# CognitiveAISystems/pogema

Measured on AMD Instinct MI355X. Metric: agent-steps/sec (whole node), 64-agent 64x64 grid, batch=8192 envs, higher is better.
Workload: dtype u32

## Files before the change

### include/pogema_amd.h

```cpp
#ifndef POGEMA_AMD_H
#define POGEMA_AMD_H

#include <stddef.h>
#include <stdint.h>

#ifdef __cplusplus
extern "C" {
#endif

#define PGX_ABI_VERSION 6

#define PGX_OK 0
#define PGX_E_INVALID (-1)
#define PGX_E_HIP (-2)
#define PGX_E_NOMEM (-3)
#define PGX_E_STATE (-4)
#define PGX_E_PLACEMENT (-5)

#define PGX_COLLISION_PRIORITY 0
#define PGX_COLLISION_BLOCK_BOTH 1
#define PGX_COLLISION_SOFT 2

#define PGX_ON_TARGET_FINISH 0
#define PGX_ON_TARGET_RESTART 1
// ... 67 lines not shown
int pgx_regenerate(pgx_env* env, const uint8_t* env_mask, float density, uint64_t seed, const uint8_t* shared_map,
                   int32_t max_retries, void* obs, void* stream);
int64_t pgx_regenerate_failures(pgx_env* env, void* stream);

int pgx_set_map_pool(pgx_env* env, const uint8_t* maps, int32_t num_maps, int32_t* capacity_out, void* stream);
int pgx_reset_pool(pgx_env* env, uint64_t seed, const uint8_t* env_mask, int32_t max_retries, void* stream);
int pgx_regenerate_pool(pgx_env* env, const uint8_t* env_mask, uint64_t seed, int32_t max_retries, void* obs,
                        void* stream);
int pgx_get_map_index(pgx_env* env, int32_t* map_index, void* stream);

int pgx_get_map(pgx_env* env, uint8_t* obstacles, void* stream);

int pgx_step(pgx_env* env, const void* actions, int action_dtype, void* obs, float* rewards,
             uint8_t* terminated, uint8_t* truncated, uint8_t* is_active, void* stream);

int pgx_xcd_shares(pgx_env* env, int32_t* shares);
int pgx_xcd_tune(pgx_env* env, void* obs, void* obs_alt, int32_t rounds, float* us_equal, float* us_tuned, void* stream);

typedef struct pgx_geometry {
    int32_t lanes_per_env;
    int32_t waves;
    int32_t envs_per_wave;
    int32_t multi_wave;
    int32_t p16;
    int32_t stagger;
    int32_t store_policy;
    int32_t state_stores;
    int32_t grid;
    int32_t lds_bytes;
    int32_t for_rollout;
// ... 142 lines not shown
```

### pogema_amd/_lib.py

```python
from __future__ import annotations

import ctypes as C
import os

_HERE = os.path.dirname(os.path.abspath(__file__))
LIB_PATH = os.environ.get("PGX_LIB") or os.path.join(_HERE, "libpogema_amd.so")

PGX_ABI_VERSION = 6

COLLISION_SYSTEMS = {"priority": 0, "block_both": 1, "soft": 2}
ON_TARGET = {"finish": 0, "restart": 1, "nothing": 2}
ACTION_DTYPES = {"int8": 0, "int32": 1, "int64": 2}
SOFT_VERTEX_RULES = {"lowest_index": 0, "all_stay": 1}
SOFT_OCCUPANCY = {"index_order": 0, "exact": 1}
COOP_REWARDS = {"all_solved": 0, "per_agent": 1}
BAD_ACTIONS = {"noop": 0, "flag": 1}
LIFELONG_RNGS = {"build": 0, "numpy": 1}
def _obs_dtypes():
    import torch
    return {torch.float32: 0, torch.uint8: 1, torch.bfloat16: 2, torch.float16: 3}


def obs_elem_bytes(dtype) -> int:
    import torch
# ... 20 lines not shown
MAX_OBS_RADIUS, MAX_AGENTS, MAX_SIDE = 15, 1024, 1024
MAX_NEIGHBOURS = 32
DIRECTIONS_FORMATS = {"float32": 0, "uint8": 1, "bits": 2}
SHIELD_TIE_BREAKS = {None: 0, "distance": 1}
MAX_PLAN_HORIZON = 256
PLAN_FIXED_PRIORITY = 1
OUTCOMES = ("STAY", "MOVED", "OBSTACLE", "SWAP", "OCCUPIED", "FOLLOW", "CONTESTED")
NUM_OUTCOMES = len(OUTCOMES)
POLICY_CHANNELS = {"obstacles": 0, "agents": 1, "target": 2, "other_goals": 3, "up": 4, "down": 5, "left": 6, "right": 7}
NUM_CHANNELS = len(POLICY_CHANNELS)
DEFAULT_POLICY_CHANNELS = ("obstacles", "agents", "target", "up", "down", "left", "right")


EXPORTED_SYMBOLS = (
    "pgx_abi_version", "pgx_last_error", "pgx_create", "pgx_check_config", "pgx_destroy", "pgx_obs_elems", "pgx_agent_elems",
    "pgx_reset_from_state", "pgx_reset_random", "pgx_regenerate", "pgx_regenerate_failures", "pgx_get_map", "pgx_step", "pgx_observe", "pgx_set_metrics_buffers", "pgx_get_state", "pgx_generate", "pgx_place_agents",
    "pgx_snapshot_bytes", "pgx_save_snapshot", "pgx_load_snapshot", "pgx_time_observe", "pgx_bad_action_count",
    "pgx_buffers_create", "pgx_buffers_ptr", "pgx_buffers_get_info", "pgx_buffers_destroy", "pgx_set_targets",
    "pgx_np_streams", "pgx_np_streams_host", "pgx_np_generate", "pgx_np_generate_host", "pgx_rollout", "pgx_buffers_stride", "pgx_buffers_drop", "pgx_xcd_shares", "pgx_xcd_tune", "pgx_buffers_create_at", "pgx_time_observe_pair", "pgx_buffers_va_reserved", "pgx_get_geometry",
    "pgx_expert_actions", "pgx_set_map_pool", "pgx_reset_pool", "pgx_regenerate_pool", "pgx_get_map_index",
    "pgx_cost_to_go", "pgx_cost_to_go_bytes", "pgx_cost_to_go_builds", "pgx_visible_agents", "pgx_pibt_actions",
    "pgx_goal_directions", "pgx_shield_actions", "pgx_pibt_plan", "pgx_move_outcomes",
    "pgx_policy_input",
)


class PgxError(RuntimeError):
    def __init__(self, code: int, message: str):
        super().__init__(f"pogema_amd engine error {code}: {message}")
        self.code = code

# ... 124 lines not shown
    lib.pgx_get_map_index.restype = C.c_int
    lib.pgx_set_targets.argtypes = [vp, vp, vp, vp]
    lib.pgx_set_targets.restype = C.c_int
    lib.pgx_bad_action_count.argtypes = [vp, vp]
    lib.pgx_bad_action_count.restype = i64
    lib.pgx_time_observe.argtypes = [vp, vp, i32, C.POINTER(C.c_float), vp]
    lib.pgx_time_observe.restype = C.c_int
    lib.pgx_time_observe_pair.argtypes = [vp, vp, vp, i32, C.POINTER(C.c_float), vp]
    lib.pgx_time_observe_pair.restype = C.c_int
    lib.pgx_snapshot_bytes.argtypes = [vp]
    lib.pgx_snapshot_bytes.restype = i64
    lib.pgx_save_snapshot.argtypes = [vp, vp, vp]
    lib.pgx_load_snapshot.argtypes = [vp, vp, vp]
    lib.pgx_save_snapshot.restype = lib.pgx_load_snapshot.restype = C.c_int
    lib.pgx_step.argtypes = [vp, vp, C.c_int, vp, vp, vp, vp, vp, vp]
    lib.pgx_observe.argtypes = [vp, vp, vp]
    lib.pgx_set_metrics_buffers.argtypes = [vp, vp, vp]
    lib.pgx_get_state.argtypes = [vp, vp, vp, vp, vp, vp, vp]
    lib.pgx_generate.argtypes = [i32, i32, i32, i32, f32, u64, i64, i32, i32, vp, vp, vp]
    lib.pgx_place_agents.argtypes = [i32, i32, i32, i32, u64, i64, i32, i32, vp, i32, vp, vp]
    for name in ("pgx_create", "pgx_destroy", "pgx_reset_from_state", "pgx_reset_random", "pgx_regenerate", "pgx_get_map",
                 "pgx_step", "pgx_observe", "pgx_set_metrics_buffers", "pgx_set_metrics_buffers",
                 "pgx_get_state", "pgx_generate", "pgx_place_agents"):
        getattr(lib, name).restype = C.c_int
    if lib.pgx_abi_version() != PGX_ABI_VERSION:
        raise ImportError(f"{LIB_PATH}: ABI version {lib.pgx_abi_version()} != expected {PGX_ABI_VERSION}; rebuild")
    _lib = lib
    return lib


# ... 5 lines not shown
```

### pogema_amd/buffers.py

```python
from __future__ import annotations

import atexit
import collections
import contextlib
import ctypes as C
import os
import threading

import numpy as np
import torch

from . import _lib

_TYPESTR = {torch.float32: "<f4", torch.uint8: "|u1", torch.float16: "<f2", torch.bfloat16: "<f2"}


class _Owner:

    def __init__(self, lib, handle):
        self._lib, self._handle = lib, handle

    def __del__(self):
        try:
            if self._handle is not None and self._handle.value:
# ... 320 lines not shown
        self._count = storage_count_hook()
        self._zone_ptrs = frozenset(int(p) for p in zone_ptrs)
        dev = obs_tensors[0].device
        n = batch * agents
        self._sets = []
        for obs in obs_tensors:
            block = torch.empty(n * 7 + 16, dtype=torch.uint8, device=dev)
            members = (obs, block[:4 * n].view(torch.float32).view(batch, agents),
                       block[4 * n:5 * n].view(torch.bool).view(batch, agents),
                       block[5 * n:6 * n].view(torch.bool).view(batch, agents),
                       block[6 * n:7 * n].view(torch.bool).view(batch, agents))
            storages = (obs.untyped_storage(), block.untyped_storage())
            self._sets.append((members, storages, tuple(st._cdata for st in storages)))
        del obs, block, members, storages
        self._idle = [tuple(self._count(c) for c in cdata) for _, _, cdata in self._sets]
        self._next = 0
        self.taken = 0
        self.misses = 0

    def __len__(self):
        return len(self._sets)

    def obs_pointers(self):
        return [members[0].data_ptr() for members, _, _ in self._sets]

    def _is_idle(self, i: int) -> bool:
        cdata, idle = self._sets[i][2], self._idle[i]
        return self._count(cdata[0]) == idle[0] and self._count(cdata[1]) == idle[1]

    def free_sets(self) -> int:
        return sum(self._is_idle(i) for i in range(len(self._sets)))

    def retire(self):
        idle = [i for i in range(len(self._sets)) if self._is_idle(i)]
        out = [self._sets[i][0][0] for i in idle if self._sets[i][0][0].data_ptr() in self._zone_ptrs]
        for i in reversed(idle):
            del self._sets[i]
            del self._idle[i]
        self._next = 0
        return out

    def take(self, with_obs: bool = True):
        n = len(self._sets)
        for k in range(n):
            i = (self._next + k) % n
            if self._is_idle(i):
                self._next = (i + 1) % n
                self.taken += 1
                m = self._sets[i][0]
                return (m[0].detach() if with_obs else None, m[1].detach(), m[2].detach(), m[3].detach(), m[4].detach())
        self.misses += 1
        return None
```

### pogema_amd/csrc/pgx_api.cpp

```cpp
#include "../../include/pogema_amd.h"

#include <hip/hip_runtime.h>

#include <algorithm>
#include <cstdarg>
#include <cstdio>
#include <cstdlib>
#include <cstring>
#include <new>
#include <string>
#include <vector>

#include "pgx_internal.h"

namespace {
thread_local std::string g_err;
}

namespace pgx {
int fail_msg(int code, const char* fmt, ...) {
    char buf[512];
    va_list ap;
    va_start(ap, fmt);
    vsnprintf(buf, sizeof buf, fmt, ap);
// ... 346 lines not shown
        alloc(e->comp_len, cells * sizeof(uint32_t));
        alloc(e->comp_cells, cells * sizeof(uint32_t));
        alloc(e->tcount, BA * sizeof(uint32_t));
        if (cfg->lifelong_rng == PGX_LIFELONG_RNG_NUMPY) {
            alloc(e->np_state, BA * sizeof(pgx::NpGen));
            alloc(e->np_state0, BA * sizeof(pgx::NpGen));
        }
    }
    if (err != hipSuccess) return fail_msg(alloc_code(err), "hipMalloc failed: %s", hipGetErrorString(err));
    err = hipMemset(e->regen_fail, 0, sizeof(uint32_t));
    if (err == hipSuccess) err = hipMemset(e->bad_count, 0, sizeof(uint32_t));
    if (err == hipSuccess && e->np_state0)
        err = pgx::launch_init_np_lifelong(e->np_state0, cfg->seed, cfg->env_index_base, cfg->batch, A, nullptr);
    if (err == hipSuccess && e->np_state0) err = hipStreamSynchronize(nullptr);
    if (err == hipSuccess) err = pgx::prepare_step(e->geo, e->geo_roll);
    if (err != hipSuccess)
        return fail_msg(PGX_E_HIP, "cannot configure the step kernel (%zu bytes of LDS): %s", e->geo.lds_bytes,
                        hipGetErrorString(err));
    if (const char* spec = getenv("PGX_XCD_WEIGHTS")) {
        float f[8], sum = 0.f;
        if (sscanf(spec, "%f,%f,%f,%f,%f,%f,%f,%f", &f[0], &f[1], &f[2], &f[3], &f[4], &f[5], &f[6], &f[7]) == 8) {
            for (float q : f) sum += q > 0.f ? q : 0.f;
            if (sum > 0.f)
                for (int x = 0; x < 8; ++x) e->xcd_w[x] = (f[x] > 0.f ? f[x] : 0.f) / sum;
        }
    }
    apply_xcd_shares(e);
    err = pgx::prepare_expert(cfg->height, cfg->width);
    if (err != hipSuccess) return fail_msg(PGX_E_HIP, "cannot configure the expert kernel: %s", hipGetErrorString(err));
    if (e->flags & 4u) {
// ... 458 lines not shown
             uint8_t* truncated, uint8_t* is_active, void* stream) {
    if (!e || !actions || !rewards || !terminated || !truncated) return fail_msg(PGX_E_INVALID, "pgx_step: null argument");
    if (const int rc = check_action_dtype("pgx_step", action_dtype)) return rc;
    DeviceGuard guard;
    if (const int rc = enter(guard, e, "pgx_step", true)) return rc;
    pgx::StepParams p = step_params(e, e->geo);
    p.mode = pgx::MODE_STEP;
    p.action_dtype = action_dtype;
    p.actions = actions;
    p.obs = static_cast<float*>(obs);
    p.rewards = rewards;
    p.terminated = terminated;
    p.truncated = truncated;
    p.act_out = is_active;
    PGX_HIP(pgx::launch_step(p, e->geo, (hipStream_t)stream));
    return PGX_OK;
}

int pgx_rollout(pgx_env* e, int32_t steps, const pgx_rollout_io* io, void* stream) {
    if (!e || !io || !io->rewards || !io->terminated || !io->truncated)
        return fail_msg(PGX_E_INVALID, "pgx_rollout: null argument");
    if (io->policy_step0 < 0 || io->policy_step0 > ((int64_t)1 << 40))
        return fail_msg(PGX_E_INVALID, "pgx_rollout: policy_step0 outside 0..2^40");
    if (steps < 1) return fail_msg(PGX_E_INVALID, "pgx_rollout: steps must be >= 1, got %d", steps);
    if (const int rc = check_action_dtype("pgx_rollout", io->action_dtype)) return rc;
    if (io->obs && io->obs_slots < 1) return fail_msg(PGX_E_INVALID, "pgx_rollout: obs given but obs_slots = %d", io->obs_slots);
    DeviceGuard guard;
    if (const int rc = enter(guard, e, "pgx_rollout", true)) return rc;
    pgx::StepParams p = step_params(e, e->geo_roll);
    p.mode = pgx::MODE_STEP;
// ... 514 lines not shown
```

### pogema_amd/csrc/pgx_internal.h

```cpp
#pragma once
#include <hip/hip_runtime.h>
#include <stddef.h>
#include <stdint.h>

namespace pgx {

int fail_msg(int code, const char* fmt, ...);

#define PGX_HIP(call)                                                                                                      \
    do {                                                                                                                   \
        const hipError_t e__ = (call);                                                                                     \
        if (e__ != hipSuccess)                                                                                             \
            return pgx::fail_msg(PGX_E_HIP, "%s failed: %s (%s:%d)", #call, hipGetErrorString(e__), __FILE__, __LINE__); \
    } while (0)

struct DeviceGuard {
    int prev = -1;
    bool changed = false;
    hipError_t err = hipSuccess;
    DeviceGuard() = default;
    explicit DeviceGuard(int dev) { (void)select(dev); }
    DeviceGuard(const DeviceGuard&) = delete;
    DeviceGuard& operator=(const DeviceGuard&) = delete;
    hipError_t select(int dev) {
// ... 95 lines not shown
    const NpGen* np_state0;
    int4* macc;
    float* metrics_out;
    uint8_t* episode_done;
    uint32_t* bad_count;
    const void* actions;
    float* obs;
    float* rewards;
    uint8_t* terminated;
    uint8_t* truncated;
    uint8_t* act_out;
    const uint8_t* only;
    unsigned long long* dbg;
};

struct RolloutParams {
    int32_t steps;
    int32_t obs_slots;
    int32_t resident_bitmap;
    int32_t reserved0;
    int64_t actions_stride;
    int64_t agents_stride;
    int64_t envs_stride;
    int64_t obs_stride;
    uint64_t policy_seed;
    int64_t policy_step0;
    int8_t* actions_out;
};

struct StepGeometry {
// ... 5 lines not shown
    int stagger;
    int store_policy;
    int state_stores;
    bool big;
    bool pc;
    bool resident_bitmap;
    size_t lds_bytes;
    int grid;
    int32_t xcd_n[8], xcd_base[8];
};
StepGeometry step_geometry(int batch, int A, int bmw, int W, bool allow_p16, int epw_override, int obs_elem_bytes,
                           int waves_override, bool for_rollout = false);
hipError_t prepare_step(const StepGeometry& g, const StepGeometry& roll);
hipError_t raise_lds_limit(const void* fn, size_t lds_bytes);
hipError_t launch_step(const StepParams& p, const StepGeometry& g, hipStream_t stream);
int xcd_partition(int blocks, const float w[8], int32_t n[8], int32_t base[8]);
hipError_t launch_rollout(const StepParams& p, const RolloutParams& rp, const StepGeometry& g, hipStream_t stream);

hipError_t launch_pack_obstacles(const uint8_t* obstacles, const uint8_t* only, uint32_t* bm, int batch, int H, int Wd,
                                 int r, int wpr, int bmw, const OutsideParams& outside, hipStream_t stream);

struct ResetParams {
    int32_t env_begin, env_count;
    int32_t H, Wd, A, r, wpr, bmw;
    int32_t lifelong;
    int32_t given_state;
    int32_t max_retries;
    uint32_t thr;
    uint64_t gen_seed;
    int64_t env_index_base;
// ... 155 lines not shown
```

### pogema_amd/csrc/pgx_kernels.hip

```cpp
#include <hip/hip_runtime.h>
#include <stdint.h>
#include <stdlib.h>

#include <array>
#include <type_traits>
#include <map>
#include <mutex>
#include <string>
#include <vector>
#include <utility>

#include "pgx_internal.h"
#include "pgx_nprng.h"

namespace pgx {

__device__ __forceinline__ uint32_t lifelong_draw(uint64_t seed, uint64_t env_index, uint32_t agent,
                                                  uint32_t counter, uint32_t n) {
    uint64_t h = gen_sm64(seed);
    h = gen_sm64(h ^ env_index);
    h = gen_sm64(h ^ (((uint64_t)agent << 32) | counter));
    return (uint32_t)(((h >> 32) * (uint64_t)n) >> 32);
}

// ... 189 lines not shown
            uint32_t m = row_bits(row) >> col;
            for (int have = W - col; have < 8; have += W) m |= row_bits(++row) << have;
            u32x4 v;
            v.x = ((m & 1u) | ((m & 2u) << 15)) * one;
            v.y = (((m >> 2) & 1u) | (((m >> 2) & 2u) << 15)) * one;
            v.z = (((m >> 4) & 1u) | (((m >> 4) & 2u) << 15)) * one;
            v.w = (((m >> 6) & 1u) | (((m >> 6) & 2u) << 15)) * one;
            if constexpr (decltype(nt_tag)::value) __builtin_nontemporal_store(v, &out4[q]);
            else out4[q] = v;
        }
    };
    if (nontemporal) loop(std::true_type{});
    else loop(std::false_type{});
}

template <int POLICY, bool PIPE>
__device__ __forceinline__ void stream_rows16_loop(f32x4_t* out4, const uint32_t* rows32, int W, int row, int col, int q0, int q1,
                                                   int qs, int last_word) {
    const int drow = (4 * qs) / W, dcol = 4 * qs - drow * W;
    if constexpr (PIPE) {
        const int fw = min(row >> 1, last_word);
        uint32_t w0 = rows32[fw], w1 = rows32[fw + 1];
        for (int q = q0; q < q1; q += qs) {
            int ncol = col + dcol, nrow = row + drow;
            if (ncol >= W) {
                ncol -= W;
                nrow += 1;
            }
            const int nw = min(nrow >> 1, last_word);
            const uint32_t n0 = rows32[nw], n1 = rows32[nw + 1];
            const uint32_t pair = (uint32_t)((((uint64_t)w1 << 32) | w0) >> (16 * (row & 1)));
            const uint32_t b = ((pair & 0xFFFFu) >> col) | ((pair >> 16) << (W - col));
            f32x4_t v;
            v.x = (float)(b & 1u);
            v.y = (float)((b >> 1) & 1u);
            v.z = (float)((b >> 2) & 1u);
            v.w = (float)((b >> 3) & 1u);
            store_obs16(&out4[q], v, (uint32_t)POLICY);
            w0 = n0;
            w1 = n1;
            row = nrow;
            col = ncol;
        }
    } else {
        for (int q = q0; q < q1; q += qs) {
            const uint32_t w0 = rows32[row >> 1], w1 = rows32[(row >> 1) + 1];
            const uint32_t pair = (uint32_t)((((uint64_t)w1 << 32) | w0) >> (16 * (row & 1)));
            const uint32_t b = ((pair & 0xFFFFu) >> col) | ((pair >> 16) << (W - col));
            f32x4_t v;
            v.x = (float)(b & 1u);
            v.y = (float)((b >> 1) & 1u);
            v.z = (float)((b >> 2) & 1u);
            v.w = (float)((b >> 3) & 1u);
            store_obs16(&out4[q], v, (uint32_t)POLICY);
            col += dcol;
// ... 17 lines not shown
        u32x4 v;
        v.x = ((m & 1u) | ((m & 2u) << 15)) * one;
        v.y = (((m >> 2) & 1u) | (((m >> 2) & 2u) << 15)) * one;
        v.z = (((m >> 4) & 1u) | (((m >> 4) & 2u) << 15)) * one;
        v.w = (((m >> 6) & 1u) | (((m >> 6) & 2u) << 15)) * one;
        store_obs16(&out4[q], __builtin_bit_cast(f32x4_t, v), (uint32_t)POLICY);
        col += dcol;
        row += drow;
        if (col >= W) {
            col -= W;
            row += 1;
        }
    }
}

template <bool PIPE>
__device__ __forceinline__ void stream_rows16_span(f32x4_t* out4, const uint32_t* rows32, int head, int W, uint32_t magic,
                                                   uint32_t spol, int q0, int q1, int qs, int last_word) {
    const int e0 = head + (q0 << 2);
    const int row = (int)__umulhi((uint32_t)e0, magic);
    const int col = e0 - row * W;
    if (spol == 0u) stream_rows16_loop<0, PIPE>(out4, rows32, W, row, col, q0, q1, qs, last_word);
    else if (spol == 1u) stream_rows16_loop<1, PIPE>(out4, rows32, W, row, col, q0, q1, qs, last_word);
    else stream_rows16_loop<2, PIPE>(out4, rows32, W, row, col, q0, q1, qs, last_word);
}
__device__ __forceinline__ void stream_rows16_edges(float* out, const uint16_t* rows16, int n, int head, int tail0, int W,
                                                    uint32_t magic, int t8) {
    if (t8 < 8) {
        const int e = (t8 < 4) ? t8 : tail0 + (t8 - 4);
        const bool mine = (t8 < 4) ? (t8 < head) : (e < n);
        if (mine) {
            const int row = (int)__umulhi((uint32_t)e, magic);
            const int col = e - row * W;
            out[e] = (float)((rows16[row] >> col) & 1u);
        }
    }
}

enum { MISC_FLAGS = 0, MISC_ARRIVED = 16, MISC_UNSOLVED = 17, MISC_OFFGOAL = 18, MISC_WORDS = 32 };

struct Carry {
    uint32_t pos = 0u, tgt = 1u;
    uint32_t ablk = 0u, anext = 0u;
    int elapsed = 0;
    int4 macc = {0, 0, 0, 0};
    bool active = false;
};
__device__ __forceinline__ uint32_t pack_action4(int a) { return (uint32_t)a <= 4u ? (uint32_t)a : 15u; }

template <int G, bool MW, bool P16, bool ROLL, bool BIG, bool PC, typename P, typename R>
__device__ __forceinline__ void step_body(P& p, R& rp, const int t, const int slot, Carry& c) {
    static_assert(!MW || G == 64, "multi-wave environments use full waves");
    static_assert(!BIG || MW, "the large-map layout runs one environment per workgroup");
    static_assert(!PC || (ROLL && !MW && P16), "the resolver / streamer pair exists for single-wave rollouts with packed rows");
    extern __shared__ __attribute__((aligned(16))) uint32_t smem[];

    const int tid = PC ? (int)(threadIdx.x & 63u) : (int)threadIdx.x;
    [[maybe_unused]] const int role = PC ? (int)(threadIdx.x >> 6) : 0;
    bool do_resolve = true;
    [[maybe_unused]] bool do_stream = true;
    if constexpr (PC) {
        do_resolve = role == 0 && t < rp.steps;
        do_stream = role == 1 && t > 0;
        if (!do_resolve && !do_stream) return;
    }
    const int NT = MW ? (int)blockDim.x : 64;
    const int lane = tid & 63;
// ... 400 lines not shown
            uint32_t b = 0u;
#pragma unroll
            for (int k = 0; k < 8; ++k) b |= pack_action4(araw[k]) << (4 * k);
            c.anext = b;
        }
      }
    }
    if (dbg && tid == 0) p.dbg[(size_t)blk * 4 + (dbg2 ? 3 : 1)] = wall_clock64();
    if (!p.obs) {
        if (late_stores) emit_state(pos, tgt, active, elapsed, macc, so);
        return;
    }
    if constexpr (PC) {
        if (!do_stream) return;
    }
    lds_sync<MW>();
    if (when_stores == 1) emit_state(pos, tgt, active, elapsed, macc, so);
    int out_slot = slot;
    if constexpr (PC) out_slot = slot == 0 ? rp.obs_slots - 1 : slot - 1;
    float* const obs_out = ROLL ? reinterpret_cast<float*>(reinterpret_cast<char*>(p.obs) + (size_t)out_slot * (size_t)rp.obs_stride) : p.obs;

    if constexpr (P16) {
        const int W_rt = W, r_rt = r;
        uint32_t* rows_base = smem;
        if constexpr (ROLL) rows_base = rp.resident_bitmap ? s_occ : smem;
        if constexpr (PC) rows_base = s_obst + epw * bmw + 2 * (epw * bmw + 2 * AS);
        auto p16_phases = [&](auto wt_tag) {
        constexpr int WT = decltype(wt_tag)::value;
        const int W = WT ? WT : W_rt;
        const int r = WT ? (WT - 1) / 2 : r_rt;
        const uint32_t wmask = (1u << W) - 1u;
        constexpr int RW = WT ? (WT + 1) / 2 : 8;
        uint32_t rp[3][RW];
#pragma unroll
        for (int t = 0; t < 3; ++t) {
#pragma unroll
            for (int m = 0; m < RW; ++m) rp[t][m] = 0u;
            const int item = tid + t * NT;
            if (item < nag * 3) {
                const int la = item / 3;
                const int c = item - la * 3;
                const int el = MW ? 0 : (p.a_magic ? (int)__umulhi((uint32_t)la, p.a_magic) : la);
                const uint32_t cell = s_apos[la];
                const int x = (int)(cell >> 16), y = (int)(cell & 0xFFFFu);
                if (c < 2) {
                    const uint32_t* bm;
                    if constexpr (BIG) bm = c == 0 ? p.obst + (size_t)env0 * bmw : s_occ;
// ... 34 lines not shown
                            asm volatile("" ::: "memory");
                        }
                    }
                } else {
                    const uint32_t tc = s_atgt[la];
                    int dx = x - (int)(tc >> 16), dy = y - (int)(tc & 0xFFFFu);
                    dx = max(-r, min(r, dx));
                    dy = max(-r, min(r, dy));
                    const int hit = r - dx;
                    const uint32_t val = (1u << (r - dy)) << (16 * (hit & 1));
#pragma unroll
                    for (int m = 0; m < RW; ++m) rp[t][m] = (m == (hit >> 1)) ? val : 0u;
                }
            }
        }
        lds_sync<MW>();
        uint16_t* rows16 = reinterpret_cast<uint16_t*>(rows_base);
#pragma unroll
        for (int t = 0; t < 3; ++t) {
            const int item = tid + t * NT;
            if (item < nag * 3) {
#pragma unroll
                for (int wy = 0; wy < (WT ? WT : 16); ++wy)
                    if (WT || wy < W) rows16[item * W + wy] = (uint16_t)(rp[t][wy >> 1] >> (16 * (wy & 1)));
            }
        }
        if (tid < 4) rows16[nag * 3 * W + tid] = 0;
        lds_sync<MW>();

        const int n = nag * 3 * W * W;
// ... 47 lines not shown
                p.dbg[(size_t)blk * 4 + 3] = wall_clock64();
            }
            return;
        }
        }
        float* out = obs_out + base;
        const int head = min(n, (int)((4 - (base & 3)) & 3));
        const uint32_t magic = p.w_magic;
        const int nvec = (n - head) >> 2;
        const int tail0 = head + (nvec << 2);
        stream_rows16_edges(out, rows16, n, head, tail0, W, magic, tid);
        if (dbg && !dbg2 && tid == 0) p.dbg[(size_t)blk * 4 + 2] = wall_clock64();
        const bool span = MW && !(p.flags & 512u);
        const int part = (nvec + nw - 1) / nw;
        const int q0 = span ? wave * part + lane : tid, q1 = span ? min(nvec, (wave + 1) * part) : nvec;
        stream_rows16_span<true>(reinterpret_cast<f32x4_t*>(out + head), reinterpret_cast<const uint32_t*>(rows16), head, W, magic,
                           (uint32_t)p.store_policy, q0, q1, span ? 64 : NT, (nag * 3 * W) >> 1);
        if (when_stores == 2) emit_state(pos, tgt, active, elapsed, macc, so);
        if (dbg && !dbg2 && tid == 0) {
            __builtin_amdgcn_s_waitcnt(0);
            p.dbg[(size_t)blk * 4 + 3] = wall_clock64();
        }
        return;
        };
        if (p.obs_u8 || p.obs_one) p16_phases(std::integral_constant<int, 0>{});
        else if (W_rt == 11) p16_phases(std::integral_constant<int, 11>{});
        else if (W_rt == 15) p16_phases(std::integral_constant<int, 15>{});
        else if (W_rt == 7) p16_phases(std::integral_constant<int, 7>{});
        else p16_phases(std::integral_constant<int, 0>{});
        return;
// ... 93 lines not shown
        if (p.store_policy == 0) stream32(std::integral_constant<uint32_t, 0u>{});
        else if (p.store_policy == 1) stream32(std::integral_constant<uint32_t, 1u>{});
        else stream32(std::integral_constant<uint32_t, 2u>{});
        if (when_stores == 2) emit_state(pos, tgt, active, elapsed, macc, so);
        if (dbg && !dbg2 && tid == 0) {
            __builtin_amdgcn_s_waitcnt(0);
            p.dbg[(size_t)blk * 4 + 3] = wall_clock64();
        }
    }
}

template <int G, bool MW, bool P16, bool BIG = false>
__global__ __launch_bounds__(MW ? 1024 : 64, MW ? 1 : 8) void step_kernel(const StepParams p) {
    const RolloutParams none{};
    Carry unused;
    step_body<G, MW, P16, false, BIG, false>(p, none, 0, 0, unused);
}

#ifndef PGX_ROLL_OCC
#define PGX_ROLL_OCC 4
#endif
template <int G, bool MW, bool P16, bool BIG = false, bool PC = false>
__global__ __launch_bounds__(MW ? 1024 : (PC ? 128 : 64), MW ? 1 : PGX_ROLL_OCC) void rollout_kernel(const StepParams p0, const RolloutParams rp0) {
    typedef const __attribute__((address_space(4))) char KC;
    typedef const __attribute__((address_space(4))) StepParams KP;
    typedef const __attribute__((address_space(4))) RolloutParams KR;
    static_assert(alignof(StepParams) == 8 && alignof(RolloutParams) == 8, "kernarg layout of rollout_kernel");
    constexpr size_t rp_offset = (sizeof(StepParams) + alignof(RolloutParams) - 1) / alignof(RolloutParams) * alignof(RolloutParams);
    const int steps = rp0.steps, slots = rp0.obs_slots;
    int slot = 0;
    Carry c;
    for (int t = 0; t < steps + (PC ? 1 : 0); ++t) {
        KC* ka = (KC*)__builtin_amdgcn_kernarg_segment_ptr();
        asm volatile("" : "+s"(ka));
        KP& p = *reinterpret_cast<KP*>(ka);
        KR& rp = *reinterpret_cast<KR*>(ka + rp_offset);
        step_body<G, MW, P16, true, BIG, PC>(p, rp, t, slot, c);
        slot = slot + 1 == slots ? 0 : slot + 1;
        if ((t & 7) == 7) c.ablk = c.anext;
        if constexpr (MW || PC) lds_sync<true>();
    }
}

__global__ void pack_obstacles_kernel(const uint8_t* __restrict__ obstacles, const uint8_t* __restrict__ only,
                                      uint32_t* __restrict__ bm, int batch, int H, int Wd, int r, int wpr, int bmw,
                                      const OutsideParams outside) {
    const size_t gid = (size_t)blockIdx.x * blockDim.x + threadIdx.x;
    const size_t total = (size_t)batch * bmw;
    if (gid >= total) return;
    const int env = (int)(gid / bmw);
    if (only && !only[env]) return;
    const int w = (int)(gid - (size_t)env * bmw);
// ... 278 lines not shown
    double acc = 0.0;
    int given = 0, grid = 0;
    for (int x = 0; x < 8; ++x) {
        acc += (double)w[x];
        int upto = x == 7 ? blocks : (int)(acc * blocks + 0.5);
        if (upto > blocks) upto = blocks;
        if (upto < given) upto = given;
        n[x] = upto - given;
        base[x] = given;
        given = upto;
        if (n[x] > grid) grid = n[x];
    }
    return grid * 8;
}

hipError_t launch_step(const StepParams& p, const StepGeometry& g, hipStream_t stream) {
    const void* fn = step_fn_for(g);
    if (!fn) return hipErrorInvalidValue;
    StepParams args = p;
    void* kargs[] = {&args};
    return hipLaunchKernel(fn, dim3(g.grid), dim3(64 * g.waves), kargs, g.lds_bytes, stream);
}


hipError_t launch_pack_obstacles(const uint8_t* obstacles, const uint8_t* only, uint32_t* bm, int batch, int H, int Wd,
                                 int r, int wpr, int bmw, const OutsideParams& outside, hipStream_t stream) {
    const size_t total = (size_t)batch * bmw;
    const int bs = 256;
    hipLaunchKernelGGL(pack_obstacles_kernel, dim3((unsigned)((total + bs - 1) / bs)), dim3(bs), 0, stream,
                       obstacles, only, bm, batch, H, Wd, r, wpr, bmw, outside);
// ... 48 lines not shown
```

### pogema_amd/vec_env.py

```python
from __future__ import annotations

import ctypes as C
import os
import warnings
from typing import Optional

import numpy as np
import torch

from . import _lib
from .grid_config import GridConfig
from .placement import PlacementMixin, choose_buffers
from .queries import QueryMixin
from .semantics import Semantics


def _as_device_index(device) -> int:
    dev = torch.device(device)
    if dev.type != "cuda":
        raise ValueError(f"VecPogema runs on a HIP device only, got {device!r}")
    return dev.index if dev.index is not None else torch.cuda.current_device()


def parse_map_pool(maps) -> torch.Tensor:
# ... 23 lines not shown
        arr = np.asarray(grid)
        if arr.dtype.kind not in "biu":
            raise ValueError(f"map_pool: map {i} holds non-integer cells ({arr.dtype})")
        if out and arr.shape != out[0].shape:
            raise ValueError(f"map_pool: map {i} is {arr.shape[0]}x{arr.shape[1]}, map 0 is "
                             f"{out[0].shape[0]}x{out[0].shape[1]}: every map of a pool has one shape")
        out.append((arr != 0).astype(np.uint8))
    return torch.from_numpy(np.ascontiguousarray(np.stack(out)))


class VecPogema(PlacementMixin, QueryMixin):

    def __init__(self, grid_config: Optional[GridConfig] = None, batch: int = 1, device="cuda:0",
                 env_index_base: int = 0, auto_reset: Optional[bool] = None, reuse_buffers="recycle",
                 obs_dtype=torch.float32, semantics: Optional[Semantics] = None,
                 placement_probe: Optional[bool] = None, placement_budget_gib=None, map_pool=None):
        self.grid_config = grid_config if grid_config is not None else GridConfig(num_agents=2)
        gc = self.grid_config
        pool = None
        if map_pool is not None:
            self._check_pool_config(gc)
            pool = parse_map_pool(map_pool)
            if (semantics if semantics is not None else Semantics.from_env()).generator_rng == "numpy":
                raise NotImplementedError("map_pool draws from the build's generator (docs/SPEC.md S10); "
                                          "generator_rng='numpy' has no pool form")
        self.observation_type = gc.observation_type
        self._possible = gc.possible_agents_xy is not None or gc.possible_targets_xy is not None
        if self._possible and (gc.possible_agents_xy is None or gc.possible_targets_xy is None or gc.map is None):
            raise ValueError("possible_agents_xy and possible_targets_xy must be given together, with an explicit `map`")
        if not 1 <= int(gc.obs_radius) <= _lib.MAX_OBS_RADIUS:
            raise ValueError(f"obs_radius={gc.obs_radius}: this engine supports 1..{_lib.MAX_OBS_RADIUS} (a window row is one "
# ... 54 lines not shown
            batch=self.batch, height=self.height, width=self.width, num_agents=self.num_agents,
            obs_radius=self.obs_radius, collision_system=_lib.COLLISION_SYSTEMS[gc.collision_system],
            on_target=_lib.ON_TARGET[gc.on_target], max_episode_steps=max(1, int(gc.max_episode_steps)),
            auto_reset=int(self.auto_reset), obs_dtype=_lib.OBS_DTYPES[self.obs_dtype], seed=int(gc.seed or 0),
            env_index_base=self.env_index_base, random_outside=0 if gc.empty_outside else 1,
            outside_density=float(gc.density), soft_vertex_rule=_lib.SOFT_VERTEX_RULES[self.semantics.soft_vertex],
            coop_reward=_lib.COOP_REWARDS[self.semantics.coop_reward],
            bad_action=_lib.BAD_ACTIONS[self.semantics.bad_action],
            lifelong_rng=_lib.LIFELONG_RNGS[self.semantics.lifelong_rng],
            soft_occupancy=_lib.SOFT_OCCUPANCY[self.semantics.soft_occupancy], abi_version=_lib.PGX_ABI_VERSION)
        self._handle = C.c_void_p()
        rc = self._lib.pgx_check_config(C.byref(cfg))
        if rc != 0:
            raise ValueError(f"this GridConfig does not fit the engine: {self._lib.pgx_last_error().decode()} (README.md, Limits)")
        _lib.check(self._lib.pgx_create(C.byref(cfg), self.device_index, C.byref(self._handle)))
        self._bufs = None
        self._buf_i = 0
        self._shared = None
        self._reset_seed = None
        self._initial = None
        self._pool = None
        self.metrics = torch.zeros((self.batch, len(_lib.METRIC_NAMES)), dtype=torch.float32, device=self.device)
        self.episode_done = torch.zeros((self.batch,), dtype=torch.bool, device=self.device)
        _lib.check(self._lib.pgx_set_metrics_buffers(self._handle, self.metrics.data_ptr(), self.episode_done.data_ptr()))
        if pool is not None:
            self.set_map_pool(pool)

    def close(self, release: bool = False):
        if getattr(self, "_handle", None) is not None and self._handle.value:
            if not release:
# ... 308 lines not shown
        if len(tensors) != (1 if self.single_buffer else 2):
            raise ValueError(f"need {1 if self.single_buffer else 2} observation tensor(s), got {len(tensors)}")
        for t in tensors:
            if t.dtype != self.obs_dtype or tuple(t.shape) != self.obs_shape or not t.is_contiguous() or t.device != self.device:
                raise ValueError(f"observation buffers must be contiguous {self.obs_dtype} tensors of shape {self.obs_shape} on {self.device}")
        self._bufs = [(obs,) + self._alloc_outputs(False)[1:] for obs in tensors]
        self._buf_i = 0
        self.placement = dict(placement or {}, adopted=True)
        if self.placement_probe and self.batch >= 2048 and self._has_state():
            self.placement.update(self.tune_xcd_shares(tensors[0], tensors[-1] if len(tensors) > 1 else None))
        return self.placement

    def _has_state(self):
        return self._initial is not None

    def _outputs(self, with_obs: bool = True):
        if self.recycle:
            return self._recycled(with_obs)
        if not self.reuse_buffers:
            return self._alloc_outputs(with_obs)
        if self._bufs is None:
            if torch.cuda.is_current_stream_capturing():
                raise RuntimeError("reuse_buffers: the output buffers are picked by a timed zone walk that synchronises "
                                   "the device -- call warm_buffers() (or one un-captured step) before capturing")
            self.warm_buffers()
        self._buf_i = 0 if self.single_buffer else self._buf_i ^ 1
        return self._bufs[self._buf_i]

    def observe(self, out: Optional[torch.Tensor] = None) -> torch.Tensor:
        if out is not None:
# ... 29 lines not shown
        for name, t, (shape, dtype) in zip(("obs", "rewards", "terminated", "truncated", "is_active"), out, want):
            if t is None and name == "obs":
                continue
            ok_dtype = t.dtype == dtype or (dtype == torch.bool and t.dtype == torch.uint8)
            if tuple(t.shape) != tuple(shape) or not ok_dtype or not t.is_contiguous() or t.device != self.device:
                raise ValueError(f"out[{name}] must be a contiguous {dtype} tensor of shape {tuple(shape)} on {self.device}")
        return out

    def step(self, actions, compute_obs: bool = True, out=None):
        actions = self._prepare_actions(actions)
        if out is not None:
            obs, rewards, terminated, truncated, is_active = self._check_out(out)
            if compute_obs and obs is None:
                raise ValueError("out[obs] is None but compute_obs=True")
        else:
            obs, rewards, terminated, truncated, is_active = self._outputs(compute_obs)
        _lib.check(self._lib.pgx_step(
            self._handle, actions.data_ptr(), self._ACTION_CODE[actions.dtype],
            obs.data_ptr() if compute_obs else None, rewards.data_ptr(), terminated.data_ptr(),
            truncated.data_ptr(), is_active.data_ptr(), self._stream()))
        if self.regenerate:
            if self._reset_seed is None:
                raise RuntimeError("auto_reset='regenerate' needs reset(seed) first (random instances)")
            if self._pool is not None:
                _lib.check(self._lib.pgx_regenerate_pool(
                    self._handle, self.episode_done.data_ptr(), self._reset_seed, 3,
                    obs.data_ptr() if compute_obs else None, self._stream()))
            else:
                if self._shared is None and self.grid_config.map is not None:
                    self._shared = self._shared_map_tensor()
                _lib.check(self._lib.pgx_regenerate(
                    self._handle, self.episode_done.data_ptr(), float(self.grid_config.density), self._reset_seed,
                    self._shared.data_ptr() if self._shared is not None else None, 3,
                    obs.data_ptr() if compute_obs else None, self._stream()))
        if self.semantics.bad_action == "flag":
            bad = int(self._lib.pgx_bad_action_count(self._handle, self._stream()))
            if bad < 0:
                _lib.check(bad)
            if bad:
                raise IndexError(f"{bad} action(s) of active agents were outside 0..{len(self.grid_config.MOVES) - 1}")
        infos = {"is_active": is_active, "episode_done": self.episode_done, "metrics": self.metrics}
        return (self._wrap_obs(obs) if compute_obs else None), rewards, terminated, truncated, infos

    def rollout(self, actions=None, obs_slots: Optional[int] = None, steps: Optional[int] = None, policy_seed: int = 0,
                policy_step0: int = 0, record_actions: bool = True):
        if self.regenerate:
            raise NotImplementedError("rollout() cannot draw new instances between its steps (auto_reset='regenerate')")
        if actions is None:
            if steps is None or int(steps) < 1:
                raise ValueError("rollout(actions=None) needs steps >= 1")
            K = int(steps)
        else:
            if not isinstance(actions, torch.Tensor):
                actions = torch.as_tensor(np.asarray(actions))
            if actions.dim() != 3 or tuple(actions.shape[1:]) != (self.batch, self.num_agents) or actions.shape[0] < 1:
                raise ValueError(f"actions must have shape [K >= 1, {self.batch}, {self.num_agents}], got {tuple(actions.shape)}")
            if steps is not None and int(steps) != int(actions.shape[0]):
# ... 116 lines not shown
```

Baseline: 4.611 billion.

## Skip rewriting unchanged zero regions of the target plane in recycled obs buffers

```diff
diff --git a/include/pogema_amd.h b/include/pogema_amd.h
--- a/include/pogema_amd.h
+++ b/include/pogema_amd.h
@@ -105,6 +105,10 @@
 int pgx_step(pgx_env* env, const void* actions, int action_dtype, void* obs, float* rewards,
              uint8_t* terminated, uint8_t* truncated, uint8_t* is_active, void* stream);
 
+int pgx_step_held(pgx_env* env, const void* actions, int action_dtype, void* obs, uint8_t* held, int32_t refresh,
+                  float* rewards, uint8_t* terminated, uint8_t* truncated, uint8_t* is_active, void* stream);
+int pgx_held_available(const pgx_env* env);
+
 int pgx_xcd_shares(pgx_env* env, int32_t* shares);
 int pgx_xcd_tune(pgx_env* env, void* obs, void* obs_alt, int32_t rounds, float* us_equal, float* us_tuned, void* stream);
 
diff --git a/pogema_amd/_lib.py b/pogema_amd/_lib.py
--- a/pogema_amd/_lib.py
+++ b/pogema_amd/_lib.py
@@ -58,7 +58,7 @@
 
 EXPORTED_SYMBOLS = (
     "pgx_abi_version", "pgx_last_error", "pgx_create", "pgx_check_config", "pgx_destroy", "pgx_obs_elems", "pgx_agent_elems",
-    "pgx_reset_from_state", "pgx_reset_random", "pgx_regenerate", "pgx_regenerate_failures", "pgx_get_map", "pgx_step", "pgx_observe", "pgx_set_metrics_buffers", "pgx_get_state", "pgx_generate", "pgx_place_agents",
+    "pgx_reset_from_state", "pgx_reset_random", "pgx_regenerate", "pgx_regenerate_failures", "pgx_get_map", "pgx_step", "pgx_step_held", "pgx_held_available", "pgx_observe", "pgx_set_metrics_buffers", "pgx_get_state", "pgx_generate", "pgx_place_agents",
     "pgx_snapshot_bytes", "pgx_save_snapshot", "pgx_load_snapshot", "pgx_time_observe", "pgx_bad_action_count",
     "pgx_buffers_create", "pgx_buffers_ptr", "pgx_buffers_get_info", "pgx_buffers_destroy", "pgx_set_targets",
     "pgx_np_streams", "pgx_np_streams_host", "pgx_np_generate", "pgx_np_generate_host", "pgx_rollout", "pgx_buffers_stride", "pgx_buffers_drop", "pgx_xcd_shares", "pgx_xcd_tune", "pgx_buffers_create_at", "pgx_time_observe_pair", "pgx_buffers_va_reserved", "pgx_get_geometry",
@@ -213,6 +213,9 @@
     lib.pgx_load_snapshot.argtypes = [vp, vp, vp]
     lib.pgx_save_snapshot.restype = lib.pgx_load_snapshot.restype = C.c_int
     lib.pgx_step.argtypes = [vp, vp, C.c_int, vp, vp, vp, vp, vp, vp]
+    lib.pgx_step_held.argtypes = [vp, vp, C.c_int, vp, vp, i32, vp, vp, vp, vp, vp]
+    lib.pgx_held_available.argtypes = [vp]
+    lib.pgx_step_held.restype = lib.pgx_held_available.restype = C.c_int
     lib.pgx_observe.argtypes = [vp, vp, vp]
     lib.pgx_set_metrics_buffers.argtypes = [vp, vp, vp]
     lib.pgx_get_state.argtypes = [vp, vp, vp, vp, vp, vp, vp]
diff --git a/pogema_amd/buffers.py b/pogema_amd/buffers.py
--- a/pogema_amd/buffers.py
+++ b/pogema_amd/buffers.py
@@ -358,6 +358,8 @@
             self._sets.append((members, storages, tuple(st._cdata for st in storages)))
         del obs, block, members, storages
         self._idle = [tuple(self._count(c) for c in cdata) for _, _, cdata in self._sets]
+        self._held = [torch.full((batch, agents), 255, dtype=torch.uint8, device=dev) for _ in self._sets]
+        self._vouched = [None] * len(self._sets)
         self._next = 0
         self.taken = 0
         self.misses = 0
@@ -381,17 +383,51 @@
         for i in reversed(idle):
             del self._sets[i]
             del self._idle[i]
+            del self._held[i]
+            del self._vouched[i]
         self._next = 0
         return out
 
-    def take(self, with_obs: bool = True):
+    def _take_index(self):
         n = len(self._sets)
         for k in range(n):
             i = (self._next + k) % n
             if self._is_idle(i):
                 self._next = (i + 1) % n
                 self.taken += 1
-                m = self._sets[i][0]
-                return (m[0].detach() if with_obs else None, m[1].detach(), m[2].detach(), m[3].detach(), m[4].detach())
+                return i
         self.misses += 1
         return None
+
+    def _hand_out(self, i: int, with_obs: bool):
+        m = self._sets[i][0]
+        return (m[0].detach() if with_obs else None, m[1].detach(), m[2].detach(), m[3].detach(), m[4].detach())
+
+    @staticmethod
+    def _version(t):
+        try:
+            return t._version
+        except Exception:
+            return None
+
+    def take(self, with_obs: bool = True):
+        i = self._take_index()
+        if i is None:
+            return None
+        if with_obs:
+            self._vouched[i] = None
+        return self._hand_out(i, with_obs)
+
+    def take_for_step(self, with_obs: bool = True):
+        i = self._take_index()
+        if i is None:
+            return None
+        trusted = False
+        if with_obs:
+            v = self._vouched[i]
+            trusted = v is not None and self._version(self._sets[i][0][0]) == v
+            self._vouched[i] = None
+        return self._hand_out(i, with_obs), self._held[i], trusted, i
+
+    def vouch(self, i: int):
+        self._vouched[i] = self._version(self._sets[i][0][0])
diff --git a/pogema_amd/csrc/pgx_api.cpp b/pogema_amd/csrc/pgx_api.cpp
--- a/pogema_amd/csrc/pgx_api.cpp
+++ b/pogema_amd/csrc/pgx_api.cpp
@@ -384,6 +384,8 @@
         err = pgx::launch_init_np_lifelong(e->np_state0, cfg->seed, cfg->env_index_base, cfg->batch, A, nullptr);
     if (err == hipSuccess && e->np_state0) err = hipStreamSynchronize(nullptr);
     if (err == hipSuccess) err = pgx::prepare_step(e->geo, e->geo_roll);
+    if (err == hipSuccess && pgx::held_available(e->geo, A, e->W, obs_elem_bytes(cfg->obs_dtype)))
+        err = pgx::prepare_step_held(e->geo, A, e->W);
     if (err != hipSuccess)
         return fail_msg(PGX_E_HIP, "cannot configure the step kernel (%zu bytes of LDS): %s", e->geo.lds_bytes,
                         hipGetErrorString(err));
@@ -872,6 +874,32 @@
     p.truncated = truncated;
     p.act_out = is_active;
     PGX_HIP(pgx::launch_step(p, e->geo, (hipStream_t)stream));
+    return PGX_OK;
+}
+
+int pgx_held_available(const pgx_env* e) {
+    if (!e) return 0;
+    return pgx::held_available(e->geo, e->cfg.num_agents, e->W, obs_elem_bytes(e->cfg.obs_dtype)) ? 1 : 0;
+}
+
+int pgx_step_held(pgx_env* e, const void* actions, int action_dtype, void* obs, uint8_t* held, int32_t refresh, float* rewards,
+                  uint8_t* terminated, uint8_t* truncated, uint8_t* is_active, void* stream) {
+    if (!e || !obs || !held || !pgx_held_available(e))
+        return pgx_step(e, actions, action_dtype, obs, rewards, terminated, truncated, is_active, stream);
+    if (!actions || !rewards || !terminated || !truncated) return fail_msg(PGX_E_INVALID, "pgx_step_held: null argument");
+    if (const int rc = check_action_dtype("pgx_step_held", action_dtype)) return rc;
+    DeviceGuard guard;
+    if (const int rc = enter(guard, e, "pgx_step_held", true)) return rc;
+    pgx::StepParams p = step_params(e, e->geo);
+    p.mode = pgx::MODE_STEP;
+    p.action_dtype = action_dtype;
+    p.actions = actions;
+    p.obs = static_cast<float*>(obs);
+    p.rewards = rewards;
+    p.terminated = terminated;
+    p.truncated = truncated;
+    p.act_out = is_active;
+    PGX_HIP(pgx::launch_step_held(p, e->geo, held, refresh != 0, (hipStream_t)stream));
     return PGX_OK;
 }
 
diff --git a/pogema_amd/csrc/pgx_internal.h b/pogema_amd/csrc/pgx_internal.h
--- a/pogema_amd/csrc/pgx_internal.h
+++ b/pogema_amd/csrc/pgx_internal.h
@@ -133,6 +133,13 @@
     unsigned long long* dbg;
 };
 
+struct HeldParams {
+    uint8_t* held;
+    int32_t refresh;
+    int32_t lds_word;
+    int32_t words;
+};
+
 struct RolloutParams {
     int32_t steps;
     int32_t obs_slots;
@@ -168,6 +175,9 @@
 hipError_t prepare_step(const StepGeometry& g, const StepGeometry& roll);
 hipError_t raise_lds_limit(const void* fn, size_t lds_bytes);
 hipError_t launch_step(const StepParams& p, const StepGeometry& g, hipStream_t stream);
+bool held_available(const StepGeometry& g, int A, int W, int obs_elem_bytes);
+hipError_t prepare_step_held(const StepGeometry& g, int A, int W);
+hipError_t launch_step_held(const StepParams& p, const StepGeometry& g, uint8_t* held, bool refresh, hipStream_t stream);
 int xcd_partition(int blocks, const float w[8], int32_t n[8], int32_t base[8]);
 hipError_t launch_rollout(const StepParams& p, const RolloutParams& rp, const StepGeometry& g, hipStream_t stream);
 
diff --git a/pogema_amd/csrc/pgx_kernels.hip b/pogema_amd/csrc/pgx_kernels.hip
--- a/pogema_amd/csrc/pgx_kernels.hip
+++ b/pogema_amd/csrc/pgx_kernels.hip
@@ -227,13 +227,20 @@
     else loop(std::false_type{});
 }
 
-template <int POLICY, bool PIPE>
+#ifndef PGX_HELD_UNIT_LOG2
+#define PGX_HELD_UNIT_LOG2 7
+#endif
+template <int POLICY, bool PIPE, bool HELD = false>
 __device__ __forceinline__ void stream_rows16_loop(f32x4_t* out4, const uint32_t* rows32, int W, int row, int col, int q0, int q1,
-                                                   int qs, int last_word) {
+                                                   int qs, int last_word, [[maybe_unused]] const uint32_t* skip = nullptr,
+                                                   [[maybe_unused]] int a0 = 0, [[maybe_unused]] int last_skip = 0) {
     const int drow = (4 * qs) / W, dcol = 4 * qs - drow * W;
+    static_assert(!HELD || PIPE, "the held stream exists in the pipelined form only");
     if constexpr (PIPE) {
         const int fw = min(row >> 1, last_word);
         uint32_t w0 = rows32[fw], w1 = rows32[fw + 1];
+        [[maybe_unused]] uint32_t sw = 0u;
+        if constexpr (HELD) sw = skip[min((q0 + a0) >> (PGX_HELD_UNIT_LOG2 + 1), last_skip)];
         for (int q = q0; q < q1; q += qs) {
             int ncol = col + dcol, nrow = row + drow;
             if (ncol >= W) {
@@ -242,16 +249,23 @@
             }
             const int nw = min(nrow >> 1, last_word);
             const uint32_t n0 = rows32[nw], n1 = rows32[nw + 1];
-            const uint32_t pair = (uint32_t)((((uint64_t)w1 << 32) | w0) >> (16 * (row & 1)));
-            const uint32_t b = ((pair & 0xFFFFu) >> col) | ((pair >> 16) << (W - col));
-            f32x4_t v;
-            v.x = (float)(b & 1u);
-            v.y = (float)((b >> 1) & 1u);
-            v.z = (float)((b >> 2) & 1u);
-            v.w = (float)((b >> 3) & 1u);
-            store_obs16(&out4[q], v, (uint32_t)POLICY);
+            [[maybe_unused]] uint32_t nsw = 0u;
+            if constexpr (HELD) nsw = skip[min((q + qs + a0) >> (PGX_HELD_UNIT_LOG2 + 1), last_skip)];
+            bool write = true;
+            if constexpr (HELD) write = !((sw >> (((q + a0) >> (PGX_HELD_UNIT_LOG2 - 4)) & 31)) & 1u);
+            if (write) {
+                const uint32_t pair = (uint32_t)((((uint64_t)w1 << 32) | w0) >> (16 * (row & 1)));
+                const uint32_t b = ((pair & 0xFFFFu) >> col) | ((pair >> 16) << (W - col));
+                f32x4_t v;
+                v.x = (float)(b & 1u);
+                v.y = (float)((b >> 1) & 1u);
+                v.z = (float)((b >> 2) & 1u);
+                v.w = (float)((b >> 3) & 1u);
+                store_obs16(&out4[q], v, (uint32_t)POLICY);
+            }
             w0 = n0;
             w1 = n1;
+            if constexpr (HELD) sw = nsw;
             row = nrow;
             col = ncol;
         }
@@ -299,15 +313,23 @@
     }
 }
 
-template <bool PIPE>
+template <bool PIPE, bool HELD = false>
 __device__ __forceinline__ void stream_rows16_span(f32x4_t* out4, const uint32_t* rows32, int head, int W, uint32_t magic,
-                                                   uint32_t spol, int q0, int q1, int qs, int last_word) {
+                                                   uint32_t spol, int q0, int q1, int qs, int last_word,
+                                                   [[maybe_unused]] const uint32_t* skip = nullptr, [[maybe_unused]] int a0 = 0,
+                                                   [[maybe_unused]] int last_skip = 0) {
     const int e0 = head + (q0 << 2);
     const int row = (int)__umulhi((uint32_t)e0, magic);
     const int col = e0 - row * W;
+    if constexpr (HELD) {
+        if (spol == 0u) stream_rows16_loop<0, PIPE, true>(out4, rows32, W, row, col, q0, q1, qs, last_word, skip, a0, last_skip);
+        else if (spol == 1u) stream_rows16_loop<1, PIPE, true>(out4, rows32, W, row, col, q0, q1, qs, last_word, skip, a0, last_skip);
+        else stream_rows16_loop<2, PIPE, true>(out4, rows32, W, row, col, q0, q1, qs, last_word, skip, a0, last_skip);
+    } else {
     if (spol == 0u) stream_rows16_loop<0, PIPE>(out4, rows32, W, row, col, q0, q1, qs, last_word);
     else if (spol == 1u) stream_rows16_loop<1, PIPE>(out4, rows32, W, row, col, q0, q1, qs, last_word);
     else stream_rows16_loop<2, PIPE>(out4, rows32, W, row, col, q0, q1, qs, last_word);
+    }
 }
 __device__ __forceinline__ void stream_rows16_edges(float* out, const uint16_t* rows16, int n, int head, int tail0, int W,
                                                     uint32_t magic, int t8) {
@@ -333,9 +355,10 @@
 };
 __device__ __forceinline__ uint32_t pack_action4(int a) { return (uint32_t)a <= 4u ? (uint32_t)a : 15u; }
 
-template <int G, bool MW, bool P16, bool ROLL, bool BIG, bool PC, typename P, typename R>
-__device__ __forceinline__ void step_body(P& p, R& rp, const int t, const int slot, Carry& c) {
+template <int G, bool MW, bool P16, bool ROLL, bool BIG, bool PC, bool HELD, typename P, typename R, typename H = int>
+__device__ __forceinline__ void step_body(P& p, R& rp, const int t, const int slot, Carry& c, [[maybe_unused]] const H& hp = H{}) {
     static_assert(!MW || G == 64, "multi-wave environments use full waves");
+    static_assert(!HELD || (P16 && !ROLL && !BIG && !PC), "the held stream exists for the packed-row single-step kernels");
     static_assert(!BIG || MW, "the large-map layout runs one environment per workgroup");
     static_assert(!PC || (ROLL && !MW && P16), "the resolver / streamer pair exists for single-wave rollouts with packed rows");
     extern __shared__ __attribute__((aligned(16))) uint32_t smem[];
@@ -766,6 +789,9 @@
     if constexpr (PC) {
         if (!do_stream) return;
     }
+    if constexpr (HELD) {
+        for (int i = tid; i < hp.words; i += NT) smem[hp.lds_word + i] = 0u;
+    }
     lds_sync<MW>();
     if (when_stores == 1) emit_state(pos, tgt, active, elapsed, macc, so);
     int out_slot = slot;
@@ -783,6 +809,10 @@
         const int r = WT ? (WT - 1) / 2 : r_rt;
         const uint32_t wmask = (1u << W) - 1u;
         constexpr int RW = WT ? (WT + 1) / 2 : 8;
+        [[maybe_unused]] uint32_t held_was = 255u;
+        if constexpr (HELD) {
+            if (tid < nag && !hp.refresh) held_was = hp.held[(size_t)env0 * A + tid];
+        }
         uint32_t rp[3][RW];
 #pragma unroll
         for (int t = 0; t < 3; ++t) {
@@ -847,6 +877,26 @@
                 }
             }
         }
+        if constexpr (HELD) {
+            if (tid < nag) {
+                const int la = tid;
+                const uint32_t cell = s_apos[la], tc = s_atgt[la];
+                const int dx = max(-r, min(r, (int)(cell >> 16) - (int)(tc >> 16)));
+                const int dy = max(-r, min(r, (int)(cell & 0xFFFFu) - (int)(tc & 0xFFFFu)));
+                const uint32_t now = (uint32_t)((r - dx) * W + (r - dy));
+                hp.held[(size_t)env0 * A + la] = (uint8_t)now;
+                if (held_was < (uint32_t)(W * W)) {
+                    constexpr int UL = PGX_HELD_UNIT_LOG2;
+                    const uintptr_t slice = reinterpret_cast<uintptr_t>(obs_out + (size_t)env0 * A * 3 * W * W);
+                    const uintptr_t plane = slice + (size_t)(la * 3 + 2) * (size_t)(W * W) * 4;
+                    const uintptr_t ub = slice >> UL;
+                    const int u1 = (int)(((plane + (size_t)(W * W) * 4) >> UL) - ub);
+                    const int uw = (int)(((plane + held_was * 4) >> UL) - ub), un = (int)(((plane + now * 4) >> UL) - ub);
+                    for (int u = (int)(((plane + ((1u << UL) - 1u)) >> UL) - ub); u < u1; ++u)
+                        if (u != uw && u != un) atomicOr(&smem[hp.lds_word + (u >> 5)], 1u << (u & 31));
+                }
+            }
+        }
         lds_sync<MW>();
         uint16_t* rows16 = reinterpret_cast<uint16_t*>(rows_base);
 #pragma unroll
@@ -924,6 +974,13 @@
         const bool span = MW && !(p.flags & 512u);
         const int part = (nvec + nw - 1) / nw;
         const int q0 = span ? wave * part + lane : tid, q1 = span ? min(nvec, (wave + 1) * part) : nvec;
+        if constexpr (HELD) {
+            const uintptr_t o4 = reinterpret_cast<uintptr_t>(out + head);
+            const int a0 = (int)((o4 >> 4) - ((reinterpret_cast<uintptr_t>(out) >> PGX_HELD_UNIT_LOG2) << (PGX_HELD_UNIT_LOG2 - 4)));
+            stream_rows16_span<true, true>(reinterpret_cast<f32x4_t*>(out + head), reinterpret_cast<const uint32_t*>(rows16), head, W,
+                                           magic, (uint32_t)p.store_policy, q0, q1, span ? 64 : NT, (nag * 3 * W) >> 1,
+                                           smem + hp.lds_word, a0, hp.words - 1);
+        } else
         stream_rows16_span<true>(reinterpret_cast<f32x4_t*>(out + head), reinterpret_cast<const uint32_t*>(rows16), head, W, magic,
                            (uint32_t)p.store_policy, q0, q1, span ? 64 : NT, (nag * 3 * W) >> 1);
         if (when_stores == 2) emit_state(pos, tgt, active, elapsed, macc, so);
@@ -1047,7 +1104,14 @@
 __global__ __launch_bounds__(MW ? 1024 : 64, MW ? 1 : 8) void step_kernel(const StepParams p) {
     const RolloutParams none{};
     Carry unused;
-    step_body<G, MW, P16, false, BIG, false>(p, none, 0, 0, unused);
+    step_body<G, MW, P16, false, BIG, false, false>(p, none, 0, 0, unused);
+}
+
+template <int G, bool MW>
+__global__ __launch_bounds__(MW ? 1024 : 64, MW ? 1 : 8) void step_held(const StepParams p, const HeldParams hp) {
+    const RolloutParams none{};
+    Carry unused;
+    step_body<G, MW, true, false, false, false, true>(p, none, 0, 0, unused, hp);
 }
 
 #ifndef PGX_ROLL_OCC
@@ -1068,7 +1132,7 @@
         asm volatile("" : "+s"(ka));
         KP& p = *reinterpret_cast<KP*>(ka);
         KR& rp = *reinterpret_cast<KR*>(ka + rp_offset);
-        step_body<G, MW, P16, true, BIG, PC>(p, rp, t, slot, c);
+        step_body<G, MW, P16, true, BIG, PC, false>(p, rp, t, slot, c);
         slot = slot + 1 == slots ? 0 : slot + 1;
         if ((t & 7) == 7) c.ablk = c.anext;
         if constexpr (MW || PC) lds_sync<true>();
@@ -1377,6 +1441,47 @@
     return grid * 8;
 }
 
+static const void* held_fn_for(const StepGeometry& g) {
+    if (g.big || !g.p16) return nullptr;
+    if (g.multi_wave) return reinterpret_cast<const void*>(&step_held<64, true>);
+#define PGX_CASE(gg) case gg: return reinterpret_cast<const void*>(&step_held<gg, false>);
+    switch (g.G) {
+        PGX_CASE(1) PGX_CASE(2) PGX_CASE(4) PGX_CASE(8) PGX_CASE(16) PGX_CASE(32) PGX_CASE(64)
+        default: return nullptr;
+    }
+#undef PGX_CASE
+}
+
+static int held_words(size_t slice_bytes) {
+    const size_t units = (slice_bytes >> PGX_HELD_UNIT_LOG2) + 2;
+    return (int)(units / 32 + 1);
+}
+
+bool held_available(const StepGeometry& g, int A, int W, int obs_elem_bytes) {
+    if (!held_fn_for(g) || obs_elem_bytes != 4 || W > 15) return false;
+    const size_t slice = (size_t)g.epw * A * 3 * W * W * 4;
+    return g.lds_bytes + (size_t)held_words(slice) * 4 <= 160 * 1024;
+}
+
+hipError_t prepare_step_held(const StepGeometry& g, int A, int W) {
+    const size_t slice = (size_t)g.epw * A * 3 * W * W * 4;
+    return raise_lds_limit(held_fn_for(g), g.lds_bytes + (size_t)held_words(slice) * 4);
+}
+
+hipError_t launch_step_held(const StepParams& p, const StepGeometry& g, uint8_t* held, bool refresh, hipStream_t stream) {
+    const void* fn = held_fn_for(g);
+    if (!fn) return hipErrorInvalidValue;
+    StepParams args = p;
+    HeldParams h;
+    const int W = 2 * p.r + 1;
+    h.held = held;
+    h.refresh = refresh ? 1 : 0;
+    h.lds_word = (int32_t)(g.lds_bytes / 4);
+    h.words = held_words((size_t)g.epw * p.num_agents * 3 * W * W * 4);
+    void* kargs[] = {&args, &h};
+    return hipLaunchKernel(fn, dim3(g.grid), dim3(64 * g.waves), kargs, g.lds_bytes + (size_t)h.words * 4, stream);
+}
+
 hipError_t launch_step(const StepParams& p, const StepGeometry& g, hipStream_t stream) {
     const void* fn = step_fn_for(g);
     if (!fn) return hipErrorInvalidValue;
diff --git a/pogema_amd/vec_env.py b/pogema_amd/vec_env.py
--- a/pogema_amd/vec_env.py
+++ b/pogema_amd/vec_env.py
@@ -61,7 +61,8 @@
     def __init__(self, grid_config: Optional[GridConfig] = None, batch: int = 1, device="cuda:0",
                  env_index_base: int = 0, auto_reset: Optional[bool] = None, reuse_buffers="recycle",
                  obs_dtype=torch.float32, semantics: Optional[Semantics] = None,
-                 placement_probe: Optional[bool] = None, placement_budget_gib=None, map_pool=None):
+                 placement_probe: Optional[bool] = None, placement_budget_gib=None, map_pool=None,
+                 held_zeros: Optional[bool] = None):
         self.grid_config = grid_config if grid_config is not None else GridConfig(num_agents=2)
         gc = self.grid_config
         pool = None
@@ -146,6 +147,13 @@
         if rc != 0:
             raise ValueError(f"this GridConfig does not fit the engine: {self._lib.pgx_last_error().decode()} (README.md, Limits)")
         _lib.check(self._lib.pgx_create(C.byref(cfg), self.device_index, C.byref(self._handle)))
+        if held_zeros is None and os.environ.get("PGX_HELD_ZEROS") in ("0", "1"):
+            held_zeros = os.environ["PGX_HELD_ZEROS"] == "1"
+        self._held_on = ((self._held_pays() if held_zeros is None else bool(held_zeros)) and self.recycle
+                         and self.obs_dtype == torch.float32 and not self.regenerate
+                         and bool(self._lib.pgx_held_available(self._handle)))
+        self._held_steps = 0
+        self._held_refreshes = 0
         self._bufs = None
         self._buf_i = 0
         self._shared = None
@@ -484,6 +492,15 @@
     def _has_state(self):
         return self._initial is not None
 
+    HELD_MIN_BYTES = 128 << 20
+
+    def _held_pays(self) -> bool:
+        return int(np.prod(self.obs_shape)) * 4 >= self.HELD_MIN_BYTES
+
+    @property
+    def held_zeros(self) -> dict:
+        return {"enabled": bool(self._held_on), "steps": self._held_steps, "refreshes": self._held_refreshes}
+
     def _outputs(self, with_obs: bool = True):
         if self.recycle:
             return self._recycled(with_obs)
@@ -543,7 +560,25 @@
             if compute_obs and obs is None:
                 raise ValueError("out[obs] is None but compute_obs=True")
         else:
-            obs, rewards, terminated, truncated, is_active = self._outputs(compute_obs)
+            held = self._held_outputs(compute_obs) if self._held_on else None
+            if held is not None:
+                (obs, rewards, terminated, truncated, is_active), record, trusted, index = held
+                if compute_obs:
+                    _lib.check(self._lib.pgx_step_held(
+                        self._handle, actions.data_ptr(), self._ACTION_CODE[actions.dtype], obs.data_ptr(), record.data_ptr(),
+                        0 if trusted else 1, rewards.data_ptr(), terminated.data_ptr(), truncated.data_ptr(),
+                        is_active.data_ptr(), self._stream()))
+                    self._recycler.vouch(index)
+                    self._held_steps += 1
+                    self._held_refreshes += 0 if trusted else 1
+                    infos = {"is_active": is_active, "episode_done": self.episode_done, "metrics": self.metrics}
+                    if self.semantics.bad_action == "flag":
+                        self._raise_on_bad_actions()
+                    return self._wrap_obs(obs), rewards, terminated, truncated, infos
+            elif self._held_on and self._recycler and not torch.cuda.is_current_stream_capturing():
+                obs, rewards, terminated, truncated, is_active = self._alloc_outputs(compute_obs)
+            else:
+                obs, rewards, terminated, truncated, is_active = self._outputs(compute_obs)
         _lib.check(self._lib.pgx_step(
             self._handle, actions.data_ptr(), self._ACTION_CODE[actions.dtype],
             obs.data_ptr() if compute_obs else None, rewards.data_ptr(), terminated.data_ptr(),
@@ -563,13 +598,24 @@
                     self._shared.data_ptr() if self._shared is not None else None, 3,
                     obs.data_ptr() if compute_obs else None, self._stream()))
         if self.semantics.bad_action == "flag":
-            bad = int(self._lib.pgx_bad_action_count(self._handle, self._stream()))
-            if bad < 0:
-                _lib.check(bad)
-            if bad:
-                raise IndexError(f"{bad} action(s) of active agents were outside 0..{len(self.grid_config.MOVES) - 1}")
+            self._raise_on_bad_actions()
         infos = {"is_active": is_active, "episode_done": self.episode_done, "metrics": self.metrics}
         return (self._wrap_obs(obs) if compute_obs else None), rewards, terminated, truncated, infos
+
+    def _raise_on_bad_actions(self):
+        bad = int(self._lib.pgx_bad_action_count(self._handle, self._stream()))
+        if bad < 0:
+            _lib.check(bad)
+        if bad:
+            raise IndexError(f"{bad} action(s) of active agents were outside 0..{len(self.grid_config.MOVES) - 1}")
+
+    def _held_outputs(self, with_obs: bool):
+        capturing = torch.cuda.is_current_stream_capturing()
+        if self._recycler is None and self._has_state() and not capturing:
+            self._recycler = self._build_recycler()
+        if not self._recycler or capturing:
+            return None
+        return self._recycler.take_for_step(with_obs)
 
     def rollout(self, actions=None, obs_slots: Optional[int] = None, steps: Optional[int] = None, policy_seed: int = 0,
                 policy_step0: int = 0, record_actions: bool = True):
```

New measurement: 5.235 billion, median of 6. +13.5%, better.
